# bcgsc/NanoSim

Measured on AMD Instinct MI355X. Metric: simulated reads/sec (genome mode, mean 8 kb), higher is better.
Workload: dtype u8

## Files before the change

nanosim_amd/csrc/nanosim_amd.hip:

```cpp
#include <hip/hip_runtime.h>
#include <hipcub/hipcub.hpp>
#include <stdio.h>
#include <stdlib.h>
#include <string.h>
#include <algorithm>
#include <chrono>
#include <atomic>
#include <condition_variable>
#include <functional>
#include <mutex>
#include <thread>
#include <type_traits>
#include <string>
#include <vector>

#include "ns_device.h"
#include "ns_materialise.h"
#include "ns_chain.h"
#include "ns_hp.h"
#include "ns_ir.h"
#include "ns_io.h"
#include "ns_pack.h"
#include "ns_cs_hist.h"
#include "ns_qual_hist.h"
// ... 201 lines not shown
        for (j = 0; j < NS_KDE_RETRY; ++j) {
            u32x4 w = ns_draw(key, ST_RATIO, 0, a, j, 0);
            double x = kde_sample(A.m.kde[NS_KDE_RATIO], w);
            if (0 <= x && x <= 1) { ratio = x; break; }
        }
        if (j == NS_KDE_RETRY) ratio = 0.5;
    }
    u32x4 ws = ns_draw(key, ST_STRAND, 0, a, 0, 0);
    ns_read rd;
    rd.rec_off = 0; rd.piece_off = piece_off; rd.n_pieces = (uint16_t)n_pieces;
    rd.reversed = (u32_to_p(ws.x) > A.m.strandness_rate) ? 1 : 0;
    if (meta_al) rd.reversed = (uint8_t)A.m_reversed;
    rd.flags = ok ? 1 : 3;
    rd.head = 0; rd.tail = 0;
    if (remainder != 0) {
        rd.head = (uint32_t)(int64_t)rint((double)remainder * ratio);
        rd.tail = (uint32_t)remainder - rd.head;
    }
    rd.seq_len = 0; rd.attempts = a;
    A.reads[r] = rd;
    cap = (cap + 3ull) & ~3ull;
    if (A.attempt > 0 && !meta_al && !trx_tab) A.l_cap[tid] = cap;
    if (A.attempt == 0 || meta_al || trx_tab) {
        A.ev_cap[r] = cap;
        if (n_pieces > 1u) A.sort_key[r] = 0x80000000u | ord_coarse(work) << 5 | ord_coarse(work0);
        else A.sort_key[r] = work > 0x7fffffffull ? 0x7fffffffu : (uint32_t)work;
        A.sort_idx[r] = (uint32_t)r;
    }
}

__device__ __forceinline__ unsigned long long wave_sum(unsigned long long v) {
    for (int off = 32; off > 0; off >>= 1) v += __shfl_xor(v, off);
    return v;
}

#ifndef NS_UCOOP_ITER
#define NS_UCOOP_ITER 3
#endif
#ifndef NS_UCOOP_MINW
#define NS_UCOOP_MINW 4
#endif
#ifndef NS_CHAIN_BLOCK
#define NS_CHAIN_BLOCK 256
#endif
#ifndef NS_CHAIN_BLOCK_BIG
#define NS_CHAIN_BLOCK_BIG 512
#endif
#define NS_PIECE_SLOTS 6u
#ifndef NS_CHAIN_MINW
#define NS_CHAIN_MINW 5
#endif
#ifdef NS_CHAIN_CLOCK
__device__ unsigned long long g_chain_clock[16];
#endif
template <bool LDS_TABLES, bool COOP, bool PIECES = false>
__global__ void __launch_bounds__(COOP ? 64 : NS_CHAIN_BLOCK_BIG, COOP ? (LDS_TABLES ? NS_UCOOP_MINW : 4) : NS_CHAIN_MINW) k_chain(GenArgs A) {
    extern __shared__ uint64_t lds_tbl[];
    CoopLds *coop = nullptr;
    if constexpr (COOP && !LDS_TABLES) { __shared__ CoopLds coop_lds; coop = &coop_lds; }
    Tabs T;
    if (LDS_TABLES) {
        const uint32_t nw = COOP ? A.m.ct.n_words_mix : A.m.ct.n_words_lds;
        for (uint32_t i = threadIdx.x; i < nw; i += blockDim.x) lds_tbl[i] = A.m.chain_blob[i];
        __syncthreads();
        T.w = lds_tbl;
    } else T.w = A.m.chain_blob;
    Tabs TM = T;
    if constexpr (COOP && !LDS_TABLES) {
        if (A.coop_mix) {
            for (uint32_t i = threadIdx.x; i < A.m.ct.n_words_mix; i += blockDim.x) lds_tbl[i] = A.m.chain_blob[i];
            __syncthreads();
            TM.w = lds_tbl;
        }
    }
    const ChainTab &ct = A.m.ct;
    const uint32_t lane = threadIdx.x & 63u;
    const uint64_t tid = COOP ? (uint64_t)blockIdx.x : (uint64_t)blockIdx.x * blockDim.x + threadIdx.x;
    const bool lead = COOP ? lane == 0 : true;
    const ns_params &prm = A.prm;
    if (!COOP && A.prio_thr) {
        uint32_t w = 0;
        if (tid < A.list_n) {
            const uint32_t k = A.sort_key[A.list[tid + (tid >= A.hole_at ? A.hole_len : 0u)]];
            w = (k >> 31) ? ord_coarse_floor((k >> 5) & 31u) : k;
        }
        for (int off = 32; off > 0; off >>= 1) w = max(w, (uint32_t)__shfl_xor((int)w, off));
        w = (uint32_t)__builtin_amdgcn_readfirstlane((int)w);
        if (w >= A.prio_thr[1]) __builtin_amdgcn_s_setprio(3);
        else if (w >= A.prio_thr[2]) __builtin_amdgcn_s_setprio(2);
        else if (w >= A.prio_thr[3]) __builtin_amdgcn_s_setprio(1);
    }
    else if (COOP || (PIECES && A.piece_mode == 1u) || blockIdx.x < (gridDim.x >> 6)) __builtin_amdgcn_s_setprio(3);
    else if (blockIdx.x < (gridDim.x >> 4)) __builtin_amdgcn_s_setprio(2);
    else if (blockIdx.x < (gridDim.x >> 2)) __builtin_amdgcn_s_setprio(1);
#ifdef NS_CHAIN_CLOCK
    const unsigned long long clk0 = wall_clock64(); uint32_t clk_multi = 0; unsigned long long clk_al = 0, clk_gap = 0, clk_pos = 0;
#endif
    unsigned long long st_over = 0, st_bases = 0, st_ref = 0, st_ev = 0;
    uint32_t st_max = 0;
    const bool piece_only = PIECES && !COOP && A.piece_mode == 1u;
    const uint32_t slot = piece_only ? (uint32_t)(tid / A.list_n) : 0u;
    const uint64_t li = piece_only ? tid % A.list_n : tid;
    if (piece_only ? slot < NS_PIECE_SLOTS : tid < A.list_n) {
        const uint64_t r = A.list ? A.list[li + (li >= A.hole_at ? A.hole_len : 0u)] : A.list_base + li;
        const int kind = (int)prm.kind;
        const bool trx_al = prm.trx && kind != NS_KIND_UNALIGNED;
        const bool meta_al = (A.meta && kind != NS_KIND_UNALIGNED) || trx_al;
        const ns_key key = make_key(A, trx_al ? trx_key_rel(A, r) : r);
        const uint32_t a = trx_al ? trx_attempt(A, r) : meta_al ? A.attempt : A.att_base[r] + A.attempt;
        ns_read rd = A.reads[r];
        const uint32_t n_pieces = rd.n_pieces;
#ifdef NS_CHAIN_CLOCK
        clk_multi = n_pieces > 1u;
#endif
        ns_piece *pc = A.pieces + rd.piece_off;
        uint32_t epoch = meta_al ? 0u : A.rstate[r] & 0xffffu, fails = meta_al ? 0u : A.rstate[r] >> 16;
        bool accepted = false, overflow = false;
        do {
            if (rd.flags & 2) { ++epoch; fails = 0; break; }
            const uint64_t ev_off = A.l_off ? A.l_base + A.l_off[tid] : A.ev_base + A.ev_off[r];
            const uint64_t ev_cap64 = A.l_off ? A.l_off[tid + 1] - A.l_off[tid] : A.ev_off[r + 1] - A.ev_off[r];
            const uint32_t ev_cap = ev_cap64 > 0xffffffffull ? 0xffffffffu : (uint32_t)ev_cap64;
            EvSink32 sink; sink.last_ins_len = 0; sink.overflow = false; sink.range = false; sink.stride = blockDim.x;
            int64_t total = (int64_t)rd.head + rd.tail;
            uint32_t evn = 0, evp = 0;
            const uint32_t trx_chrom = trx_al ? pc[0].pos : 0u;
            const uint32_t pi_lo = piece_only ? slot : 0u, pi_hi = (piece_only && slot + 1u < NS_PIECE_SLOTS) ? min(slot + 1u, n_pieces) : n_pieces;
            for (uint32_t pi = pi_lo; pi < pi_hi; ++pi) {
                ns_piece p = pc[pi];
                if (PIECES && !COOP && A.piece_mode == 2u) {
                    const uint32_t fl = (uint32_t)(p.ref_gpos >> 32);
                    if (fl & 1u) sink.range = true;
                    if (fl & 2u) sink.overflow = true;
                    p.ev_off = ev_off + p.ev_off;
                    pc[pi] = p;
                    evn += p.n_ev;
                    if (!p.kind) total += (int64_t)(int32_t)(uint32_t)p.ref_gpos;
                    continue;
                }
                if (piece_only) {
                    evp = (uint32_t)p.ev_off;
                    const uint32_t end = pi + 1u < n_pieces ? (uint32_t)pc[pi + 1u].ev_off : ev_cap;
                    sink.range = false; sink.overflow = false;
                    sink.ev = A.events + ev_off + evp; sink.cap = end > evp ? end - evp : 0u;
                }
                const int32_t m32 = (int32_t)p.ref_len;
                const uint32_t sid = p.kind ? NS_GAP_SEG + (pi >> 1) : (pi >> 1);
                if (!piece_only) { sink.ev = A.events + ev_off + evp; sink.cap = ev_cap > evp ? ev_cap - evp : 0; }
                sink.n = 0; sink.shift = 0;
// ... 116 lines not shown
            }
            if (!pos_ok || (!A.hp && !trx_al && (seq_len < prm.min_len || seq_len > prm.max_len))) { ++epoch; fails = 0; break; }
            rd.flags = 0; rd.seq_len = (uint32_t)seq_len; rd.attempts = a;
            uint32_t nl = 0; bool first = true;
            for (uint32_t pi = 0; pi < n_pieces; ++pi) {
                ns_piece p = pc[pi];
                if (p.kind && kind == NS_KIND_ALIGNED) {
                    if (A.meta) nl += 5 + dec_digits(p.out_len);
                    continue;
                }
                if (!first) nl += 2;
                first = false;
                nl += (A.ref.name_off[p.chrom + 1] - A.ref.name_off[p.chrom] - 1) + 1 + dec_digits(p.pos) + dec_digits(p.ref_len);
            }
            nl += (kind == NS_KIND_UNALIGNED ? 11u : 9u) + (meta_al ? 0u : dec_digits(A.name_first + r)) + ir_name;
            if (kind == NS_KIND_ALIGNED && n_pieces > 1) nl += 9;
            nl += 2  + 1 + dec_digits(rd.head) + 1 + 1 + dec_digits(rd.tail + polya);
            uint64_t err_len = 0;
            if (prm.emit_errlog && !A.errlen_later) {
                for (uint32_t pi = 0; pi < n_pieces; ++pi) {
                    ns_piece p = pc[pi];
                    if (p.kind) continue;
                    const ns_event *ev = A.events + p.ev_off;
                    for (uint32_t j = 0; j < p.n_ev; ++j) {
                        ns_event e = ev[j];
                        err_len += nl + dec_digits(e.pos) + dec_digits(ns_ev_len(e.info)) + 2u * ns_ev_len(e.info) + 9u;
                    }
                }
            }
            if (lead) {
                A.name_len[r] = (uint16_t)nl;
                A.rec_len[r] = prm.emit_records ? (uint64_t)nl + 2 + (uint64_t)seq_len + 1 + (prm.fastq ? (uint64_t)seq_len + 3 : 0) : 0;
                A.err_len[r] = err_len;
                if (A.polya) A.polya[r] = (uint16_t)polya;
                if (A.ir_need) A.ir_need[r] = spliced ? ir_slot_bytes(pc[0].ref_len) : 0;
                if (meta_al) { A.accept[r] = 1ull | (uint64_t)n_pieces << 32; A.sort_key[r] = evn; }
                st_bases = A.hp ? 0ull : (unsigned long long)seq_len; st_ref = ref_bases; st_ev = evn; st_max = (uint32_t)seq_len;
                if (trx_al) st_bases = st_ref = st_ev = 0;
            }
            accepted = true;
        } while (false);
        if (lead && !piece_only) {
            if (overflow) st_over += 1;
            A.reads[r] = rd;
            if (meta_al) {  }
            else if (accepted) A.att_base[r] = a;
            if (!meta_al && !accepted && !overflow) {
                A.rstate[r] = (epoch & 0xffffu) | fails << 16;
                A.next_list[atomicAdd(A.next_n, 1u)] = (uint32_t)r;
            }
        }
    }
#ifdef NS_CHAIN_CLOCK
    if (!COOP && A.attempt == 0) {
        const unsigned long long dt = wall_clock64() - clk0;
        const bool any_multi = __ballot(clk_multi != 0) != 0;
        if ((threadIdx.x & 63) == 0) { unsigned long long *C = g_chain_clock + (any_multi ? 4 : 0); atomicMax(&C[0], dt); atomicAdd(&C[1], dt); atomicAdd(&C[2], 1ull);
                                       atomicMax(&C[3], (unsigned long long)blockIdx.x << 32 | dt);
                                       if (any_multi) { atomicAdd(&g_chain_clock[8], clk_al); atomicAdd(&g_chain_clock[9], clk_gap); atomicAdd(&g_chain_clock[10], clk_pos ? wall_clock64() - clk_pos : 0ull); } }
    }
#endif
    st_over = wave_sum(st_over); st_bases = wave_sum(st_bases); st_ref = wave_sum(st_ref); st_ev = wave_sum(st_ev);
    if (A.prm.kind == NS_KIND_UNALIGNED) for (int off = 32; off > 0; off >>= 1) st_max = max(st_max, (uint32_t)__shfl_xor((int)st_max, off));
    if ((threadIdx.x & 63) == 0) {
        unsigned long long *S = ns_stats_way(A.stats, blockIdx.x & (NS_STATS_WAYS - 1u));
        if (st_over) atomicAdd(&S[NS_STAT_OVER], st_over);
        if (st_bases) atomicAdd(&S[NS_STAT_BASES], st_bases);
        if (st_ref) atomicAdd(&S[NS_STAT_REF_BASES], st_ref);
        if (st_ev) atomicAdd(&S[NS_STAT_EVENTS], st_ev);
        if (A.prm.kind == NS_KIND_UNALIGNED && st_max) atomicMax(&S[NS_STAT_MAX_READ], (unsigned long long)st_max);
    }
}

__global__ void __launch_bounds__(64) k_stats_fold(unsigned long long *stats, uint32_t *zero_me) {
    if (threadIdx.x == 0 && zero_me) *zero_me = 0;
    unsigned long long *S = ns_stats_way(stats, threadIdx.x);
    constexpr int MAX = NS_STAT_MAX_READ;
    unsigned long long v[MAX + 1];
    #pragma unroll
    for (int k = 0; k <= MAX; ++k) { v[k] = S[k]; S[k] = 0; }
    #pragma unroll
    for (int k = 0; k < MAX; ++k) v[k] = wave_sum(v[k]);
    for (int off = 32; off > 0; off >>= 1) { const unsigned long long o = __shfl_xor(v[MAX], off); v[MAX] = o > v[MAX] ? o : v[MAX]; }
    if (threadIdx.x == 0) {
        #pragma unroll
        for (int k = 0; k < MAX; ++k) if (v[k]) atomicAdd(&stats[k], v[k]);
        if (v[MAX]) atomicMax(&stats[MAX], v[MAX]);
    }
}

#define NS_ORD_BINS 2048u
__device__ __forceinline__ uint32_t ord_bin(uint32_t key31) {
    if (key31 >> 31) return 1023u - (key31 & 1023u);
    const uint32_t key = key31;
    uint32_t v = key;
    if (key >= 32u) { const uint32_t e = 31u - (uint32_t)__clz((int)key); v = (e - 4u) * 32u + ((key >> (e - 5u)) & 31u); }
    return 1024u + 1023u - v;
}
__global__ void __launch_bounds__(1024) k_order_hist(const uint32_t *__restrict__ keys, uint32_t n, uint32_t *__restrict__ hist) {
    __shared__ uint32_t h[NS_ORD_BINS];
    h[threadIdx.x] = 0; h[threadIdx.x + 1024u] = 0;
    __syncthreads();
    for (uint32_t i = blockIdx.x * 1024u + threadIdx.x; i < n; i += gridDim.x * 1024u) atomicAdd(&h[ord_bin(keys[i])], 1u);
    __syncthreads();
    if (h[threadIdx.x]) atomicAdd(&hist[threadIdx.x], h[threadIdx.x]);
    if (h[threadIdx.x + 1024u]) atomicAdd(&hist[threadIdx.x + 1024u], h[threadIdx.x + 1024u]);
// ... 2649 lines not shown
                    n_coop = (cur_n - std::min(cur_n, n_multi)) >> kn.coop_shift;
                const uint32_t coop_at = (a == 0 && prm->kind == NS_KIND_ALIGNED) ? std::min(cur_n, n_multi) : 0u;
                uint32_t m_coop = 0;
                if (coop_at && n_coop) {
                    const bool piece_threads = lds && !kn.no_piece_threads;
                    const uint32_t sh = piece_threads ? (kn.coop_shift > 1u ? kn.coop_shift - 1u : 0u) : (kn.coop_shift > 5u ? kn.coop_shift - 5u : 0u);
                    m_coop = std::min(coop_at, std::max(coop_at >> sh, 64u));
                }
                if (n_coop) {
                    GenArgs B = A; B.list_n = n_coop + m_coop; B.list = cur + (m_coop ? 0u : coop_at);
                    if (m_coop) { B.hole_at = m_coop; B.hole_len = coop_at - m_coop; }
                    B.coop_k1 = kn.ucoop_k1 ? 1u : 0u;
                    if ((rc = launch_chain_coop(ctx, B, st))) return rc;
                    if (coop_at) { A.list = cur + m_coop; A.hole_at = coop_at - m_coop; A.hole_len = n_coop; } else A.list = cur + n_coop;
                    A.list_n = cur_n - n_coop - m_coop;
                }
                uint32_t n_pt = 0;
                if (a == 0 && lds && n_coop && coop_at > m_coop && !kn.no_piece_threads) {
                    if (!ctx->stream3) {
                        HIPCHK(hipStreamCreateWithFlags(&ctx->stream3, hipStreamNonBlocking));
                        HIPCHK(hipEventCreateWithFlags(&ctx->ev_join3, hipEventDisableTiming));
                    }
                    n_pt = coop_at - m_coop;
                    const uint32_t cb = ctx->chain_block;
                    GenArgs P = A; P.list = cur + m_coop; P.list_n = n_pt; P.hole_at = 0; P.hole_len = 0; P.prio_thr = nullptr;
                    const size_t lds_p = ctx->lds_bytes + (P.ev_stage ? cb * 32u : 0u);
                    HIPCHK(hipStreamWaitEvent(ctx->stream3, ctx->ev_fork, 0));
                    P.piece_mode = 1;
                    k_chain<true, false, true><<<dim3((unsigned)(((uint64_t)n_pt * NS_PIECE_SLOTS + cb - 1) / cb)), dim3(cb), lds_p, ctx->stream3>>>(P);
                    P.piece_mode = 2;
                    k_chain<true, false, true><<<dim3((n_pt + cb - 1) / cb), dim3(cb), lds_p, ctx->stream3>>>(P);
                    HIPCHK(hipGetLastError());
                    HIPCHK(hipEventRecord(ctx->ev_join3, ctx->stream3));
                    A.list = cur + coop_at + n_coop; A.hole_at = 0; A.hole_len = 0; A.list_n = cur_n - coop_at - n_coop;
                }
                if (a == 0 && n_multi && !n_pt && prm->kind == NS_KIND_ALIGNED) A.prio_thr = ctx->ord_bins.view<const uint32_t>() + 2 * NS_ORD_BINS;
                if ((rc = launch_chain(ctx, A, st))) return rc;
                if (n_coop) HIPCHK(hipStreamWaitEvent(st, ctx->ev_join, 0));
                if (n_pt) HIPCHK(hipStreamWaitEvent(st, ctx->ev_join3, 0));
                HIPCHK(hipEventRecord(ctx->evt[EV_CHAIN_END], st));
                if (ctx->gate_signal) ctx->gate_signal->store(1, std::memory_order_release);
                if ((rc = end_pass(ctx, A, retry, stats, ms_chain, info, overflow))) return rc;
                if (overflow) break;
                cur_n = (uint32_t)(stats[NS_STAT_NEXT_N] & 0xffffffffull);
                if (!cur_n) { pl.tot_cap = used; break; }
                if (a + 1 >= NS_MAX_ATTEMPT) return attempt_limit(ctx);
                cur = nxt; nxt = cur == list_b ? list_c : list_b;
            }
            info->ms_kernel[NS_K_EVENTS] = ms_chain;
#ifdef NS_CHAIN_CLOCK
            if (prm->kind == NS_KIND_ALIGNED) { unsigned long long c[16], z[16] = {0}; HIPCHK(hipMemcpyFromSymbol(c, HIP_SYMBOL(g_chain_clock), sizeof c)); HIPCHK(hipMemcpyToSymbol(HIP_SYMBOL(g_chain_clock), z, sizeof z));
              fprintf(stderr, "chain clock: lane 0 of the multi waves: aligned pieces %.3f ms, gaps %.3f ms, behind the lists %.3f ms (means) | ", c[6] ? c[8] * 1e-5 / c[6] : 0.0, c[6] ? c[9] * 1e-5 / c[6] : 0.0, c[6] ? c[10] * 1e-5 / c[6] : 0.0);
              fprintf(stderr, "chain clock: single waves %llu max %.3f ms mean %.3f ms (the group's last block: %llu) | multi waves %llu max %.3f ms mean %.3f ms (the group's last block: %llu) | ms_chain %.3f\n",
                  c[2], c[0] * 1e-5, c[2] ? c[1] * 1e-5 / c[2] : 0.0, c[3] >> 32, c[6], c[4] * 1e-5, c[6] ? c[5] * 1e-5 / c[6] : 0.0, c[7] >> 32, ms_chain); }
#endif
            if (!overflow) break;
        }
        if (A.ir_need && (rc = ir_splice(ctx, A, n))) return rc;
        if (!A.hp) break;
        if ((rc = hp_stage1(ctx, prm, A, n, pl.tot_pieces, stats, &pl.ms_hp))) return rc;
        if (!stats[NS_STAT_HP_FAILED]) break;
        if (hp_round >= (int)NS_MAX_ATTEMPT) return fail(ctx, NS_EINVAL, "reads keep failing the final length check in -k mode");
        A.keep_state = 1;
    }
    return NS_OK;
}

static int check_params(ns_ctx *ctx, const ns_params *prm) {
    if (!ctx->has_model || !ctx->has_ref) return fail(ctx, NS_ESTATE, "ns_generate before ns_load_model/ns_set_reference");
    if (prm->kind > NS_KIND_PERFECT) return fail(ctx, NS_EINVAL, "bad kind");
    if (prm->emit_records > NS_EMIT_SIZES) return fail(ctx, NS_EINVAL, "bad emit_records");
    if (prm->kind != NS_KIND_PERFECT && !(ctx->m.flags & NS_MODEL_HAS_ERRORS)) return fail(ctx, NS_EINVAL, "model has no error tables");
    if (prm->kind == NS_KIND_UNALIGNED && !prm->use_lognormal && !(ctx->m.flags & NS_MODEL_HAS_UNALIGNED))
        return fail(ctx, NS_EINVAL, "model has no unaligned-length KDE");
    if (prm->fastq && !(ctx->m.flags & NS_MODEL_HAS_QUALS)) return fail(ctx, NS_EINVAL, "model has no quality tables");
    if (prm->chimeric && !(ctx->m.flags & NS_MODEL_HAS_CHIMERIC)) return fail(ctx, NS_EINVAL, "model has no chimeric tables");
    if (prm->kmer_bias && prm->kind == NS_KIND_ALIGNED && !(ctx->m.flags & NS_MODEL_HAS_HP))
        return fail(ctx, NS_EINVAL, "-k needs the homopolymer model (-hp)");
    const bool meta_al = prm->meta && prm->kind != NS_KIND_UNALIGNED;
    if (prm->meta) {
        if (!ctx->nspecies) return fail(ctx, NS_ESTATE, "metagenome batch before ns_set_species");
        if (prm->kind == NS_KIND_PERFECT && prm->chimeric) return fail(ctx, NS_EINVAL, "perfect reads cannot be chimeric");
        if (meta_al && !ctx->has_abun) return fail(ctx, NS_ESTATE, "metagenome batch before ns_set_abundance");
        if (meta_al && prm->chimeric && !ctx->has_inflated) return fail(ctx, NS_EINVAL, "chimeric metagenome batch needs abun_inflated");
    }
    if (prm->trx) {
        if (!ctx->has_trx) return fail(ctx, NS_ESTATE, "transcriptome batch before ns_set_transcriptome");
        if (prm->meta || prm->chimeric || prm->use_lognormal) return fail(ctx, NS_EINVAL, "transcriptome batches are neither metagenome nor chimeric nor log-normal");
        if (prm->kind != NS_KIND_UNALIGNED && !(ctx->m.flags & NS_MODEL_HAS_KDE2D)) return fail(ctx, NS_EINVAL, "model has no 2-D KDE (_aligned_region_2d)");
    }
    if (prm->model_ir) {
        if (!prm->trx) return fail(ctx, NS_EINVAL, "model_ir is a transcriptome option");
        if (!ctx->has_ir) return fail(ctx, NS_ESTATE, "model_ir batch before ns_set_intron_retention");
    }
    if (prm->n_reads > 0x7ffffff0ull) return fail(ctx, NS_EINVAL, "batch too large (split into several calls)");
    if (prm->first_read + prm->n_reads >= (1ull << 40)) return fail(ctx, NS_EINVAL, "read index exceeds 2^40");
    return NS_OK;
}

static int batch_args(ns_ctx *ctx, const ns_params *prm, size_t n, GenArgs &A) {
    int rc;
    if ((rc = ensure_all(ctx, {{ctx->n_pieces, n + 1}, {ctx->piece_off, n + 1}, {ctx->ev_cap, n + 1}, {ctx->ev_off, n + 1},
                               {ctx->l_cap, n + 1}, {ctx->l_off, n + 1}, {ctx->rec_len, n + 1}, {ctx->rec_off, n + 1},
                               {ctx->err_len, n + 1}, {ctx->err_off, n + 1}, {ctx->name_len, n + 1}, {ctx->reads, n},
                               {ctx->stats, NS_STATS_BYTES}, {ctx->sort_key, n + 1}, {ctx->sort_idx, n + 1}, {ctx->sort_key_out, n + 1},
                               {ctx->order, n + 1}, {ctx->list_b, (n + 1) * 4}, {ctx->list_c, (n + 1) * 4}, {ctx->rstate, n + 1},
                               {ctx->att_base, n + 1}, {ctx->scr_len, n + 1}, {ctx->scr_off, n + 1}})))
// ... 514 lines not shown
```

nanosim_amd/csrc/ns_chain.h:

```cpp
#pragma once
#include "ns_device.h"

struct Tabs {
    const uint64_t *w;
    NS_DEV const double *d(uint32_t off) const { return reinterpret_cast<const double *>(w + off); }
    NS_DEV const uint64_t *q(uint32_t off) const { return w + off; }
    NS_DEV const uint16_t *h(uint32_t off) const { return reinterpret_cast<const uint16_t *>(w + off); }
    NS_DEV const uint32_t *u(uint32_t off) const { return reinterpret_cast<const uint32_t *>(w + off); }
    NS_DEV const int32_t *i(uint32_t off) const { return reinterpret_cast<const int32_t *>(w + off); }
};

template <class V>
NS_DEV int32_t ecdf_lookup_g(const double *__restrict__ hi, const V *__restrict__ vhi, uint32_t n,
                                                 double vlo0, const uint16_t *__restrict__ guide, uint32_t u) {
    double p = u32_to_p(u);
    uint32_t s = guide[guide_cell(u)];
    if (s < n) {
        const double h0 = hi[s], h1 = hi[min(s + 1, n - 1)];
        if (p > h0) {
            ++s;
            if (s < n && p > h1) { ++s; while (s < n && p > hi[s]) ++s; }
        }
    }
    if (s >= n) { s = n - 1; p = hi[s]; }
// ... 490 lines not shown
                        if (st - 1 > Lk) { ty[k][2] = NS_MIS; ln[k][2] = st - 1 - Lk; ne = 3; }
                    }
                } else {
                    if (!Lk) { ty[k][0] = NS_DEL; ln[k][0] = st; ne = 1; }
                    else {
                        ty[k][0] = NS_DEL; ln[k][0] = st > Lk ? st - Lk : 1u; ne = 1;
                        if (Lk > st - 1) { ty[k][1] = NS_INS; ln[k][1] = Lk - (st - 1); ne = 2; }
                    }
                }
            }
            bad |= ln[k][0] > NS_EV_LEN_MAX || ln[k][1] > NS_EV_LEN_MAX || ln[k][2] > NS_EV_LEN_MAX;
            ln[k][0] = min(ln[k][0], NS_EV_LEN_MAX); ln[k][1] = min(ln[k][1], NS_EV_LEN_MAX); ln[k][2] = min(ln[k][2], NS_EV_LEN_MAX);
            n_ev[k] = ne; n_loc[k] = n_lane; n_lane += ne;
        }
        const uint32_t d_incl = wave_incl_scan(d_lane);
        const uint32_t ne_incl = wave_incl_scan(n_lane | n_exec_l << 16);
        const uint32_t d_front = d_incl - d_lane, n_front = (ne_incl & 0xffffu) - n_lane;
        auto dsh = [](uint32_t t, uint32_t l) { return t == NS_INS ? l : t == NS_DEL ? 0u - l : 0u; };
        #pragma unroll
        for (int k = 0; k < K; ++k) {
            if (!n_ev[k]) continue;
            const uint32_t sh = (uint32_t)s.shift + (pend0 + (i_incl - i_lane) + i_loc[k] - L[k]) - (d_front + d_loc[k]);
            const uint32_t d0 = dsh(ty[k][0], ln[k][0]), d1 = n_ev[k] > 1 ? dsh(ty[k][1], ln[k][1]) : 0u;
            if (!ev_shift_fits((int32_t)sh) || (n_ev[k] > 1 && !ev_shift_fits((int32_t)(sh + d0))) || (n_ev[k] > 2 && !ev_shift_fits((int32_t)(sh + d0 + d1)))) bad = true;
            const uint32_t slot = s.n + n_front + n_loc[k];
            if (slot < s.cap) { ns_event e; e.pos = ps[k][0]; e.info = ns_ev_pack(ln[k][0], ty[k][0], (int32_t)sh); s.ev[slot] = e; }
            if (n_ev[k] > 1 && slot + 1 < s.cap) { ns_event e; e.pos = ps[k][1]; e.info = ns_ev_pack(ln[k][1], ty[k][1], (int32_t)(sh + d0)); s.ev[slot + 1] = e; }
            if (n_ev[k] > 2 && slot + 2 < s.cap) { ns_event e; e.pos = ps[k][2]; e.info = ns_ev_pack(ln[k][2], ty[k][2], (int32_t)(sh + d0 + d1)); s.ev[slot + 2] = e; }
        }
        const uint32_t ne_tot = (uint32_t)__builtin_amdgcn_readlane((int)ne_incl, 63);
        const uint32_t n_blk = ne_tot & 0xffffu, n_ran = ne_tot >> 16;
        const uint32_t del_tot = (uint32_t)__builtin_amdgcn_readlane((int)d_incl, 63), ins_tot = (uint32_t)__builtin_amdgcn_readlane((int)i_incl, 63);
        uint32_t adv_tot = (uint32_t)__builtin_amdgcn_readlane((int)a_incl, 63);
        if (n_ran < 64u * K) adv_tot = (uint32_t)__builtin_amdgcn_readlane((int)wave_incl_scan(a_exec), 63);
        if (s.n + n_blk > s.cap) s.overflow = true;
        s.n += n_blk;
        l_new += (int32_t)ins_tot - (int32_t)del_tot;
        uint32_t pend1 = pend0 + ins_tot;
        if (HAS) {
            const int jl = 63 - __clzll((long long)HAS);
            pend1 = (uint32_t)__shfl((int)run, jl) + ins_tot - (uint32_t)__shfl((int)i_incl, jl);
        }
        s.shift = (int32_t)((uint32_t)s.shift + (pend0 + ins_tot - pend1) - del_tot);
        pend0 = pend1;
        pos0 += adv_tot;
        if (n_ran < 64u * K || pos0 >= (uint32_t)m_ref) break;
    }
    if (__ballot(bad)) s.range = true;
    if ((int32_t)pos0 > middle_ref) { l_new += (int32_t)pos0 - middle_ref; middle_ref = (int32_t)pos0; }
    return EList32{l_new, middle_ref};
}

#define COOP_MAX_BINS 16u
struct CoopLds {
    uint32_t err_tab[64];
    uint16_t step_tab[64][4];
    uint32_t match_tab[64][COOP_MAX_BINS];
    ns_event ev_buf[64];
};

__device__ inline EList32 coop_error_list(const Tabs &TM, const Tabs &T, const ChainTab &c, int32_t m_ref, const ns_key &key, uint32_t seg,
                                          uint32_t attempt, EvSink32 &s, CoopLds &S, uint32_t lane) {
    int32_t l_new = m_ref, pos = 0, middle_ref = m_ref;
    int state = NS_ST_START;
    u32x4 w = ns_draw(key, ST_EVENT, seg, attempt, 0, 0);
    int32_t prev_match = ecdf_lookup_g(T.d(c.fm_hi), T.d(c.fm_vhi), c.fm_n, c.fm_vlo0, T.h(c.fm_guide), w.x);
    if (prev_match < 2) prev_match = 2;
    pos += prev_match;
    uint32_t it0 = 1;
    int32_t last_ins_pos = -1;
    const uint64_t *trans = TM.q(c.trans);
    const int32_t *bins = T.i(c.mm_bin);
    const uint32_t *seg_off = T.u(c.mm_seg_off);
    const uint8_t *bin_lut = reinterpret_cast<const uint8_t *>(T.w + c.mm_bin_lut);
    auto bin_of = [&](int32_t v) -> uint32_t {
        if ((uint32_t)v < 256u) return bin_lut[v];
        uint32_t b = 0;
        for (; b < c.mm_nbins; ++b)
            if (bins[2 * b] <= v && v < bins[2 * b + 1]) break;
        return b >= c.mm_nbins ? c.mm_nbins - 1 : b;
    };
    uint32_t pbin = bin_of(prev_match);
    while (pos < middle_ref) {
        {
            const u32x4 wi = ns_draw(key, ST_EVENT, seg, attempt, it0 + lane, 0);
            uint32_t eb = 0;
#pragma unroll
            for (int st = 0; st < 7; ++st) eb |= (uint32_t)trans_pick_u(trans + 3 * st, wi.x) << (2 * st);
            S.err_tab[lane] = eb;
#pragma unroll
            for (int t = 0; t < 3; ++t) S.step_tab[lane][t] = (uint16_t)run_length_t(TM, c, t, wi.y, wi.z);
            if (c.int_image) {
                const uint16_t *g16 = T.h(c.mm_g16);
                const uint64_t *gvf = T.q(c.mm_gv_full);
                const uint32_t cell = wi.w >> 16, nb = c.mm_nbins;
                const uint64_t uu = wi.w;
                for (uint32_t b0 = 0; b0 < nb; b0 += 4) {
                    uint32_t o[4], nc[4], s0[4];
                    uint64_t ga[4], gb[4];
#pragma unroll
                    for (uint32_t k = 0; k < 4; ++k) {
                        const uint32_t b = min(b0 + k, nb - 1u);
                        o[k] = seg_off[b]; nc[k] = seg_off[b + 1] - o[k];
                        s0[k] = g16[(size_t)b * 65536u + cell];
                    }
#pragma unroll
                    for (uint32_t k = 0; k < 4; ++k) {
                        const uint32_t sc = min(s0[k], nc[k] ? nc[k] - 1u : 0u);
                        ga[k] = gvf[o[k] + sc]; gb[k] = gvf[o[k] + sc + 1u];
                    }
#pragma unroll
                    for (uint32_t k = 0; k < 4; ++k) {
                        const uint32_t b = min(b0 + k, nb - 1u);
                        const uint32_t k0 = (s0[k] < nc[k] ? 1u : 0u) & (uu >= NS_G_THR(ga[k]) ? 1u : 0u);
                        const uint32_t k1 = k0 & (s0[k] + 1u < nc[k] ? 1u : 0u) & (uu >= NS_G_THR(gb[k]) ? 1u : 0u);
                        const uint64_t g = k0 ? gb[k] : ga[k];
                        int32_t v = (int32_t)(uint32_t)(g >> 35) - 1;
                        if (!((s0[k] + k0 < nc[k]) && !k1 && (g & NS_GV_UNIT)))
                            v = ecdf_lookup_gv(gvf + o[k], nc[k], T.h(c.mm_guide) + NS_GUIDE_CELLS * b, wi.w, T.q(c.sub2_full), T.d(c.mm_hi) + o[k], T.d(c.mm_vhi) + o[k], T.d(c.mm_vlo0)[b]);
                        if (b0 + k < nb) S.match_tab[lane][b0 + k] = (uint32_t)(uint16_t)v | bin_of(v) << 16 | bin_of(v == 0 ? 1 : v) << 24;
                    }
                }
            } else
            for (uint32_t b = 0; b < c.mm_nbins; ++b) {
                const uint32_t o = seg_off[b];
                const int32_t v = ecdf_lookup_g(T.d(c.mm_hi) + o, T.d(c.mm_vhi) + o, seg_off[b + 1] - o, T.d(c.mm_vlo0)[b], T.h(c.mm_guide) + NS_GUIDE_CELLS * b, wi.w);
                S.match_tab[lane][b] = (uint32_t)(uint16_t)v | bin_of(v) << 16 | bin_of(v == 0 ? 1 : v) << 24;
            }
        }
        __builtin_amdgcn_fence(__ATOMIC_ACQ_REL, "wavefront");
        __builtin_amdgcn_wave_barrier();
        uint32_t nl = 0;
        uint32_t i = 0;
        for (; i < 64 && pos < middle_ref; ++i) {
            const int error = (int)((S.err_tab[i] >> (2 * state)) & 3u);
            int32_t step = S.step_tab[i][error];
            if (error == NS_INS) l_new += step; else if (error == NS_DEL) l_new -= step;
            int32_t epos = pos;
            if (error != NS_INS) {
                pos += step;
                if (pos >= middle_ref) { l_new += pos - middle_ref; middle_ref = pos; }
            } else {
                if (last_ins_pos == pos && (nl > 0 || s.n > 0)) {
                    if (nl > 0) --nl; else --s.n;
                    s.shift -= (int32_t)s.last_ins_len;
                }
                last_ins_pos = pos;
            }
            {
                const uint32_t l = step > (int32_t)NS_EV_LEN_MAX ? NS_EV_LEN_MAX : (uint32_t)step;
                if (step > (int32_t)NS_EV_LEN_MAX || !ev_shift_fits(s.shift)) s.range = true;
                ns_event e; e.pos = (uint32_t)epos; e.info = ns_ev_pack(l, (uint32_t)error, s.shift);
                if (lane == 0) S.ev_buf[nl] = e;
                ++nl;
                if (error == NS_INS) { s.shift += (int32_t)l; s.last_ins_len = l; } else if (error == NS_DEL) s.shift -= (int32_t)l;
            }
            state = NS_ST_MIS + error;
            const uint32_t me = S.match_tab[i][pbin];
            step = (int32_t)(me & 0xffffu);
            pbin = (me >> 16) & 0xffu;
            if (prev_match == 0 && step == 0) { step = 1; pbin = me >> 24; }
            prev_match = step;
            if (pos + prev_match > middle_ref) { l_new += pos + prev_match - middle_ref; middle_ref = pos + prev_match; }
            pos += prev_match;
            if (prev_match == 0) state += 3;
            else last_ins_pos = -1;
        }
        __builtin_amdgcn_fence(__ATOMIC_ACQ_REL, "wavefront");
        __builtin_amdgcn_wave_barrier();
        if (lane < nl) {
            if (s.n + lane < s.cap) s.ev[s.n + lane] = S.ev_buf[lane];
        }
        if (s.n + nl > s.cap) s.overflow = true;
        s.n += nl;
        it0 += i;
        __builtin_amdgcn_fence(__ATOMIC_ACQ_REL, "wavefront");
        __builtin_amdgcn_wave_barrier();
    }
    return EList32{l_new, middle_ref};
}
```

Before: 126.5 million.

## Walk cooperative error list from VGPR lanes via readlane instead of LDS

Restructures the wave-per-read error-list generation. Each lane still evaluates one speculative row into LDS, but the serial walk now reads rows through register readlane from a transposed per-lane copy, and buffers events in lane registers instead of an LDS event buffer. The step table is packed into two words per row. The aim is to cut LDS round-trips and barriers on the serial critical path, at the cost of more register pressure and a 16-way unrolled walk. Clock instrumentation for the cooperative path is also added behind a debug macro.

```diff
diff --git a/nanosim_amd/csrc/nanosim_amd.hip b/nanosim_amd/csrc/nanosim_amd.hip
--- a/nanosim_amd/csrc/nanosim_amd.hip
+++ b/nanosim_amd/csrc/nanosim_amd.hip
@@ -277,6 +277,8 @@
 #endif
 #ifdef NS_CHAIN_CLOCK
 __device__ unsigned long long g_chain_clock[16];
+#define NS_COOP_CLOCK_N 4096u
+__device__ unsigned long long g_coop_clock[NS_COOP_CLOCK_N][4];
 #endif
 template <bool LDS_TABLES, bool COOP, bool PIECES = false>
 __global__ void __launch_bounds__(COOP ? 64 : NS_CHAIN_BLOCK_BIG, COOP ? (LDS_TABLES ? NS_UCOOP_MINW : 4) : NS_CHAIN_MINW) k_chain(GenArgs A) {
@@ -320,6 +322,7 @@
     else if (blockIdx.x < (gridDim.x >> 2)) __builtin_amdgcn_s_setprio(1);
 #ifdef NS_CHAIN_CLOCK
     const unsigned long long clk0 = wall_clock64(); uint32_t clk_multi = 0; unsigned long long clk_al = 0, clk_gap = 0, clk_pos = 0;
+    if constexpr (COOP && !LDS_TABLES) { if (lane == 0) coop->clk[0] = coop->clk[1] = coop->clk[2] = coop->clk[3] = 0; }
 #endif
     unsigned long long st_over = 0, st_bases = 0, st_ref = 0, st_ev = 0;
     uint32_t st_max = 0;
@@ -542,6 +545,9 @@
         }
     }
 #ifdef NS_CHAIN_CLOCK
+    if constexpr (COOP && !LDS_TABLES) {
+        if (lane == 0 && A.attempt == 0 && blockIdx.x < NS_COOP_CLOCK_N) for (int k = 0; k < 4; ++k) g_coop_clock[blockIdx.x][k] = coop->clk[k];
+    }
     if (!COOP && A.attempt == 0) {
         const unsigned long long dt = wall_clock64() - clk0;
         const bool any_multi = __ballot(clk_multi != 0) != 0;
@@ -3297,7 +3303,12 @@
             if (prm->kind == NS_KIND_ALIGNED) { unsigned long long c[16], z[16] = {0}; HIPCHK(hipMemcpyFromSymbol(c, HIP_SYMBOL(g_chain_clock), sizeof c)); HIPCHK(hipMemcpyToSymbol(HIP_SYMBOL(g_chain_clock), z, sizeof z));
               fprintf(stderr, "chain clock: lane 0 of the multi waves: aligned pieces %.3f ms, gaps %.3f ms, behind the lists %.3f ms (means) | ", c[6] ? c[8] * 1e-5 / c[6] : 0.0, c[6] ? c[9] * 1e-5 / c[6] : 0.0, c[6] ? c[10] * 1e-5 / c[6] : 0.0);
               fprintf(stderr, "chain clock: single waves %llu max %.3f ms mean %.3f ms (the group's last block: %llu) | multi waves %llu max %.3f ms mean %.3f ms (the group's last block: %llu) | ms_chain %.3f\n",
-                  c[2], c[0] * 1e-5, c[2] ? c[1] * 1e-5 / c[2] : 0.0, c[3] >> 32, c[6], c[4] * 1e-5, c[6] ? c[5] * 1e-5 / c[6] : 0.0, c[7] >> 32, ms_chain); }
+                  c[2], c[0] * 1e-5, c[2] ? c[1] * 1e-5 / c[2] : 0.0, c[3] >> 32, c[6], c[4] * 1e-5, c[6] ? c[5] * 1e-5 / c[6] : 0.0, c[7] >> 32, ms_chain);
+              static unsigned long long cc[NS_COOP_CLOCK_N][4]; HIPCHK(hipMemcpyFromSymbol(cc, HIP_SYMBOL(g_coop_clock), sizeof cc));
+              uint32_t w = 0; for (uint32_t k = 1; k < NS_COOP_CLOCK_N; ++k) if (cc[k][3] > cc[w][3]) w = k;
+              fprintf(stderr, "coop clock: wave-per-read wavefront %u with the most iterations (%llu): speculative %.3f ms, walk %.3f ms, flush %.3f ms\n",
+                  w, cc[w][3], cc[w][0] * 1e-5, cc[w][1] * 1e-5, cc[w][2] * 1e-5);
+              static const unsigned long long zz[NS_COOP_CLOCK_N][4] = {}; HIPCHK(hipMemcpyToSymbol(HIP_SYMBOL(g_coop_clock), zz, sizeof zz)); }
 #endif
             if (!overflow) break;
         }
diff --git a/nanosim_amd/csrc/ns_chain.h b/nanosim_amd/csrc/ns_chain.h
--- a/nanosim_amd/csrc/ns_chain.h
+++ b/nanosim_amd/csrc/ns_chain.h
@@ -566,97 +566,121 @@
 }
 
 #define COOP_MAX_BINS 16u
+#define COOP_ROW_RA 16u
+#define COOP_ROW_RB 17u
+#define COOP_ROW_WORDS 19u
 struct CoopLds {
-    uint32_t err_tab[64];
-    uint16_t step_tab[64][4];
-    uint32_t match_tab[64][COOP_MAX_BINS];
-    ns_event ev_buf[64];
+    uint32_t match_tab[64][COOP_ROW_WORDS];
+#ifdef NS_CHAIN_CLOCK
+    unsigned long long clk[4], clk_t;
+#endif
 };
-
-__device__ inline EList32 coop_error_list(const Tabs &TM, const Tabs &T, const ChainTab &c, int32_t m_ref, const ns_key &key, uint32_t seg,
-                                          uint32_t attempt, EvSink32 &s, CoopLds &S, uint32_t lane) {
-    int32_t l_new = m_ref, pos = 0, middle_ref = m_ref;
-    int state = NS_ST_START;
-    u32x4 w = ns_draw(key, ST_EVENT, seg, attempt, 0, 0);
-    int32_t prev_match = ecdf_lookup_g(T.d(c.fm_hi), T.d(c.fm_vhi), c.fm_n, c.fm_vlo0, T.h(c.fm_guide), w.x);
-    if (prev_match < 2) prev_match = 2;
-    pos += prev_match;
-    uint32_t it0 = 1;
-    int32_t last_ins_pos = -1;
+#ifdef NS_CHAIN_CLOCK
+#define NS_COOP_CLK(S, lane, k) do { if ((lane) == 0) { const unsigned long long t_ = wall_clock64(); (S).clk[k] += t_ - (S).clk_t; (S).clk_t = t_; } } while (0)
+#else
+#define NS_COOP_CLK(S, lane, k) do { } while (0)
+#endif
+
+NS_DEV uint32_t coop_bin_of(const Tabs &T, const ChainTab &c, int32_t v) {
+    if ((uint32_t)v < 256u) return reinterpret_cast<const uint8_t *>(T.w + c.mm_bin_lut)[v];
+    const int32_t *bins = T.i(c.mm_bin);
+    uint32_t b = 0;
+    for (; b < c.mm_nbins; ++b)
+        if (bins[2 * b] <= v && v < bins[2 * b + 1]) break;
+    return b >= c.mm_nbins ? c.mm_nbins - 1 : b;
+}
+NS_DEV uint32_t coop_match_word(const Tabs &T, const ChainTab &c, int32_t v) {
+    return (uint32_t)(uint16_t)v | coop_bin_of(T, c, v) << 16 | coop_bin_of(T, c, v == 0 ? 1 : v) << 24;
+}
+
+NS_DEV void coop_eval_row(const Tabs &TM, const Tabs &T, const ChainTab &c, const ns_key &key, uint32_t seg, uint32_t attempt, uint32_t it,
+                          uint32_t *row) {
     const uint64_t *trans = TM.q(c.trans);
-    const int32_t *bins = T.i(c.mm_bin);
     const uint32_t *seg_off = T.u(c.mm_seg_off);
-    const uint8_t *bin_lut = reinterpret_cast<const uint8_t *>(T.w + c.mm_bin_lut);
-    auto bin_of = [&](int32_t v) -> uint32_t {
-        if ((uint32_t)v < 256u) return bin_lut[v];
-        uint32_t b = 0;
-        for (; b < c.mm_nbins; ++b)
-            if (bins[2 * b] <= v && v < bins[2 * b + 1]) break;
-        return b >= c.mm_nbins ? c.mm_nbins - 1 : b;
-    };
-    uint32_t pbin = bin_of(prev_match);
-    while (pos < middle_ref) {
-        {
-            const u32x4 wi = ns_draw(key, ST_EVENT, seg, attempt, it0 + lane, 0);
-            uint32_t eb = 0;
+    const u32x4 wi = ns_draw(key, ST_EVENT, seg, attempt, it, 0);
+    uint32_t eb = 0;
 #pragma unroll
-            for (int st = 0; st < 7; ++st) eb |= (uint32_t)trans_pick_u(trans + 3 * st, wi.x) << (2 * st);
-            S.err_tab[lane] = eb;
+    for (int st = 0; st < 7; ++st) eb |= (uint32_t)trans_pick_u(trans + 3 * st, wi.x) << (2 * st);
+    row[COOP_ROW_RA] = eb | (uint32_t)(uint16_t)run_length_t(TM, c, NS_MIS, wi.y, wi.z) << 16;
+    row[COOP_ROW_RB] = (uint32_t)(uint16_t)run_length_t(TM, c, NS_INS, wi.y, wi.z) | (uint32_t)(uint16_t)run_length_t(TM, c, NS_DEL, wi.y, wi.z) << 16;
+    if (c.int_image) {
+        const uint16_t *g16 = T.h(c.mm_g16);
+        const uint64_t *gvf = T.q(c.mm_gv_full);
+        const uint32_t cell = wi.w >> 16, nb = c.mm_nbins;
+        const uint64_t uu = wi.w;
+        for (uint32_t b0 = 0; b0 < nb; b0 += 4) {
+            uint32_t o[4], nc[4], s0[4];
+            uint64_t ga[4], gb[4];
 #pragma unroll
-            for (int t = 0; t < 3; ++t) S.step_tab[lane][t] = (uint16_t)run_length_t(TM, c, t, wi.y, wi.z);
-            if (c.int_image) {
-                const uint16_t *g16 = T.h(c.mm_g16);
-                const uint64_t *gvf = T.q(c.mm_gv_full);
-                const uint32_t cell = wi.w >> 16, nb = c.mm_nbins;
-                const uint64_t uu = wi.w;
-                for (uint32_t b0 = 0; b0 < nb; b0 += 4) {
-                    uint32_t o[4], nc[4], s0[4];
-                    uint64_t ga[4], gb[4];
+            for (uint32_t k = 0; k < 4; ++k) {
+                const uint32_t b = min(b0 + k, nb - 1u);
+                o[k] = seg_off[b]; nc[k] = seg_off[b + 1] - o[k];
+                s0[k] = g16[(size_t)b * 65536u + cell];
+            }
 #pragma unroll
-                    for (uint32_t k = 0; k < 4; ++k) {
-                        const uint32_t b = min(b0 + k, nb - 1u);
-                        o[k] = seg_off[b]; nc[k] = seg_off[b + 1] - o[k];
-                        s0[k] = g16[(size_t)b * 65536u + cell];
-                    }
+            for (uint32_t k = 0; k < 4; ++k) {
+                const uint32_t sc = min(s0[k], nc[k] ? nc[k] - 1u : 0u);
+                ga[k] = gvf[o[k] + sc]; gb[k] = gvf[o[k] + sc + 1u];
+            }
 #pragma unroll
-                    for (uint32_t k = 0; k < 4; ++k) {
-                        const uint32_t sc = min(s0[k], nc[k] ? nc[k] - 1u : 0u);
-                        ga[k] = gvf[o[k] + sc]; gb[k] = gvf[o[k] + sc + 1u];
-                    }
-#pragma unroll
-                    for (uint32_t k = 0; k < 4; ++k) {
-                        const uint32_t b = min(b0 + k, nb - 1u);
-                        const uint32_t k0 = (s0[k] < nc[k] ? 1u : 0u) & (uu >= NS_G_THR(ga[k]) ? 1u : 0u);
-                        const uint32_t k1 = k0 & (s0[k] + 1u < nc[k] ? 1u : 0u) & (uu >= NS_G_THR(gb[k]) ? 1u : 0u);
-                        const uint64_t g = k0 ? gb[k] : ga[k];
-                        int32_t v = (int32_t)(uint32_t)(g >> 35) - 1;
-                        if (!((s0[k] + k0 < nc[k]) && !k1 && (g & NS_GV_UNIT)))
-                            v = ecdf_lookup_gv(gvf + o[k], nc[k], T.h(c.mm_guide) + NS_GUIDE_CELLS * b, wi.w, T.q(c.sub2_full), T.d(c.mm_hi) + o[k], T.d(c.mm_vhi) + o[k], T.d(c.mm_vlo0)[b]);
-                        if (b0 + k < nb) S.match_tab[lane][b0 + k] = (uint32_t)(uint16_t)v | bin_of(v) << 16 | bin_of(v == 0 ? 1 : v) << 24;
-                    }
-                }
-            } else
-            for (uint32_t b = 0; b < c.mm_nbins; ++b) {
-                const uint32_t o = seg_off[b];
-                const int32_t v = ecdf_lookup_g(T.d(c.mm_hi) + o, T.d(c.mm_vhi) + o, seg_off[b + 1] - o, T.d(c.mm_vlo0)[b], T.h(c.mm_guide) + NS_GUIDE_CELLS * b, wi.w);
-                S.match_tab[lane][b] = (uint32_t)(uint16_t)v | bin_of(v) << 16 | bin_of(v == 0 ? 1 : v) << 24;
+            for (uint32_t k = 0; k < 4; ++k) {
+                const uint32_t b = min(b0 + k, nb - 1u);
+                const uint32_t k0 = (s0[k] < nc[k] ? 1u : 0u) & (uu >= NS_G_THR(ga[k]) ? 1u : 0u);
+                const uint32_t k1 = k0 & (s0[k] + 1u < nc[k] ? 1u : 0u) & (uu >= NS_G_THR(gb[k]) ? 1u : 0u);
+                const uint64_t g = k0 ? gb[k] : ga[k];
+                int32_t v = (int32_t)(uint32_t)(g >> 35) - 1;
+                if (!((s0[k] + k0 < nc[k]) && !k1 && (g & NS_GV_UNIT)))
+                    v = ecdf_lookup_gv(gvf + o[k], nc[k], T.h(c.mm_guide) + NS_GUIDE_CELLS * b, wi.w, T.q(c.sub2_full), T.d(c.mm_hi) + o[k], T.d(c.mm_vhi) + o[k], T.d(c.mm_vlo0)[b]);
+                if (b0 + k < nb) row[b0 + k] = coop_match_word(T, c, v);
             }
         }
-        __builtin_amdgcn_fence(__ATOMIC_ACQ_REL, "wavefront");
-        __builtin_amdgcn_wave_barrier();
-        uint32_t nl = 0;
-        uint32_t i = 0;
-        for (; i < 64 && pos < middle_ref; ++i) {
-            const int error = (int)((S.err_tab[i] >> (2 * state)) & 3u);
-            int32_t step = S.step_tab[i][error];
+    } else
+    for (uint32_t b = 0; b < c.mm_nbins; ++b) {
+        const uint32_t o = seg_off[b];
+        const int32_t v = ecdf_lookup_g(T.d(c.mm_hi) + o, T.d(c.mm_vhi) + o, seg_off[b + 1] - o, T.d(c.mm_vlo0)[b], T.h(c.mm_guide) + NS_GUIDE_CELLS * b, wi.w);
+        row[b] = coop_match_word(T, c, v);
+    }
+}
+
+NS_DEV uint32_t coop_tr_row(uint32_t lane, uint32_t r) { return 16u * (lane >> 4) + r; }
+NS_DEV uint32_t coop_tr_col(uint32_t lane) { return lane & 15u; }
+
+#ifndef NS_COOP_COUNT
+#define NS_COOP_COUNT(what)
+#endif
+enum { NS_CCNT_POP_EARLIER, NS_CCNT_ZERO_RULE };
+struct CoopChain {
+    int32_t l_new, pos, middle_ref, prev_match, last_ins_pos;
+    uint32_t state, pbin;
+};
+template <uint32_t N> struct CoopIdx { static constexpr uint32_t value = N; };
+template <class W>
+struct CoopRows {
+    typename W::Reg ra, rb;
+    typename W::Reg col[COOP_MAX_BINS];
+};
+template <class W>
+NS_DEV uint32_t coop_walk_block(const CoopRows<W> &R, CoopChain &k, EvSink32 &s, typename W::Reg &ev_pos, typename W::Reg &ev_info, uint32_t &nl_out) {
+    int32_t l_new = k.l_new, pos = k.pos, middle_ref = k.middle_ref, prev_match = k.prev_match, last_ins_pos = k.last_ins_pos;
+    uint32_t state = k.state, pbin = k.pbin;
+    uint32_t nl = 0;
+    uint32_t n_it = 0;
+    auto one = [&](uint32_t g, auto rc) __attribute__((always_inline)) -> bool {
+            constexpr uint32_t r = decltype(rc)::value;
+            if (pos >= middle_ref) return false;
+            const uint32_t i = g + r;
+            const uint32_t wa = W::rd(R.ra, i), wb = W::rd(R.rb, i);
+            const uint32_t me = W::rd(R.col[r], g + pbin);
+            const int error = (int)((wa >> (2u * state)) & 3u);
+            int32_t step = (int32_t)(error == NS_MIS ? wa >> 16 : error == NS_INS ? wb & 0xffffu : wb >> 16);
             if (error == NS_INS) l_new += step; else if (error == NS_DEL) l_new -= step;
-            int32_t epos = pos;
+            const int32_t epos = pos;
             if (error != NS_INS) {
                 pos += step;
                 if (pos >= middle_ref) { l_new += pos - middle_ref; middle_ref = pos; }
             } else {
                 if (last_ins_pos == pos && (nl > 0 || s.n > 0)) {
-                    if (nl > 0) --nl; else --s.n;
+                    if (nl > 0) --nl; else { --s.n; NS_COOP_COUNT(NS_CCNT_POP_EARLIER); }
                     s.shift -= (int32_t)s.last_ins_len;
                 }
                 last_ins_pos = pos;
@@ -664,32 +688,92 @@
             {
                 const uint32_t l = step > (int32_t)NS_EV_LEN_MAX ? NS_EV_LEN_MAX : (uint32_t)step;
                 if (step > (int32_t)NS_EV_LEN_MAX || !ev_shift_fits(s.shift)) s.range = true;
-                ns_event e; e.pos = (uint32_t)epos; e.info = ns_ev_pack(l, (uint32_t)error, s.shift);
-                if (lane == 0) S.ev_buf[nl] = e;
+                W::wr(ev_pos, nl, (uint32_t)epos);
+                W::wr(ev_info, nl, ns_ev_pack(l, (uint32_t)error, s.shift));
                 ++nl;
                 if (error == NS_INS) { s.shift += (int32_t)l; s.last_ins_len = l; } else if (error == NS_DEL) s.shift -= (int32_t)l;
             }
-            state = NS_ST_MIS + error;
-            const uint32_t me = S.match_tab[i][pbin];
+            state = NS_ST_MIS + (uint32_t)error;
             step = (int32_t)(me & 0xffffu);
             pbin = (me >> 16) & 0xffu;
-            if (prev_match == 0 && step == 0) { step = 1; pbin = me >> 24; }
+            if (prev_match == 0 && step == 0) { step = 1; pbin = me >> 24; NS_COOP_COUNT(NS_CCNT_ZERO_RULE); }
             prev_match = step;
             if (pos + prev_match > middle_ref) { l_new += pos + prev_match - middle_ref; middle_ref = pos + prev_match; }
             pos += prev_match;
             if (prev_match == 0) state += 3;
             else last_ins_pos = -1;
-        }
+            ++n_it;
+            return true;
+    };
+    for (uint32_t g = 0; g < 64u; g += 16u)
+        if (!(one(g, CoopIdx<0>{}) && one(g, CoopIdx<1>{}) && one(g, CoopIdx<2>{}) && one(g, CoopIdx<3>{}) && one(g, CoopIdx<4>{}) && one(g, CoopIdx<5>{}) &&
+              one(g, CoopIdx<6>{}) && one(g, CoopIdx<7>{}) && one(g, CoopIdx<8>{}) && one(g, CoopIdx<9>{}) && one(g, CoopIdx<10>{}) && one(g, CoopIdx<11>{}) &&
+              one(g, CoopIdx<12>{}) && one(g, CoopIdx<13>{}) && one(g, CoopIdx<14>{}) && one(g, CoopIdx<15>{}))) break;
+    k.l_new = l_new; k.pos = pos; k.middle_ref = middle_ref; k.prev_match = prev_match; k.last_ins_pos = last_ins_pos;
+    k.state = state; k.pbin = pbin;
+    nl_out = nl;
+    return n_it;
+}
+NS_DEV void coop_flush_lane(const EvSink32 &s, uint32_t nl, uint32_t lane, uint32_t pos, uint32_t info) {
+    if (lane < nl && s.n + lane < s.cap) { ns_event e; e.pos = pos; e.info = info; s.ev[s.n + lane] = e; }
+}
+NS_DEV void coop_flush_close(EvSink32 &s, uint32_t nl) {
+    if (s.n + nl > s.cap) s.overflow = true;
+    s.n += nl;
+}
+NS_DEV CoopChain coop_chain_open(const Tabs &T, const ChainTab &c, int32_t m_ref, const ns_key &key, uint32_t seg, uint32_t attempt) {
+    CoopChain k;
+    k.l_new = m_ref; k.pos = 0; k.middle_ref = m_ref; k.state = NS_ST_START; k.last_ins_pos = -1;
+    const u32x4 w = ns_draw(key, ST_EVENT, seg, attempt, 0, 0);
+    k.prev_match = ecdf_lookup_g(T.d(c.fm_hi), T.d(c.fm_vhi), c.fm_n, c.fm_vlo0, T.h(c.fm_guide), w.x);
+    if (k.prev_match < 2) k.prev_match = 2;
+    k.pos += k.prev_match;
+    k.pbin = coop_bin_of(T, c, k.prev_match);
+    return k;
+}
+
+#ifndef NS_HOST_TEST
+struct CoopWave {
+    typedef uint32_t Reg;
+    static __device__ __forceinline__ uint32_t rd(Reg v, uint32_t lane) { return (uint32_t)__builtin_amdgcn_readlane((int)v, (int)lane); }
+    static __device__ __forceinline__ void wr(Reg &v, uint32_t lane, uint32_t x) {
+        v = __builtin_amdgcn_mbcnt_hi(~0u, __builtin_amdgcn_mbcnt_lo(~0u, 0u)) == lane ? x : v;
+    }
+};
+__device__ __forceinline__ int32_t coop_uni(int32_t v) { return __builtin_amdgcn_readfirstlane(v); }
+
+__device__ inline EList32 coop_error_list(const Tabs &TM, const Tabs &T, const ChainTab &c, int32_t m_ref, const ns_key &key, uint32_t seg,
+                                          uint32_t attempt, EvSink32 &s, CoopLds &S, uint32_t lane) {
+    CoopChain k = coop_chain_open(T, c, m_ref, key, seg, attempt);
+    k.l_new = coop_uni(k.l_new); k.pos = coop_uni(k.pos); k.middle_ref = coop_uni(k.middle_ref); k.prev_match = coop_uni(k.prev_match);
+    k.pbin = (uint32_t)coop_uni((int32_t)k.pbin);
+    s.n = (uint32_t)coop_uni((int32_t)s.n); s.shift = coop_uni(s.shift); s.last_ins_len = (uint32_t)coop_uni((int32_t)s.last_ins_len);
+    uint32_t it0 = 1;
+#ifdef NS_CHAIN_CLOCK
+    if (lane == 0) S.clk_t = wall_clock64();
+#endif
+    while (k.pos < k.middle_ref) {
+        CoopRows<CoopWave> R;
+        coop_eval_row(TM, T, c, key, seg, attempt, it0 + lane, S.match_tab[lane]);
         __builtin_amdgcn_fence(__ATOMIC_ACQ_REL, "wavefront");
         __builtin_amdgcn_wave_barrier();
-        if (lane < nl) {
-            if (s.n + lane < s.cap) s.ev[s.n + lane] = S.ev_buf[lane];
-        }
-        if (s.n + nl > s.cap) s.overflow = true;
-        s.n += nl;
-        it0 += i;
+        R.ra = S.match_tab[lane][COOP_ROW_RA]; R.rb = S.match_tab[lane][COOP_ROW_RB];
+#pragma unroll
+        for (uint32_t r = 0; r < COOP_MAX_BINS; ++r) R.col[r] = S.match_tab[coop_tr_row(lane, r)][coop_tr_col(lane)];
         __builtin_amdgcn_fence(__ATOMIC_ACQ_REL, "wavefront");
         __builtin_amdgcn_wave_barrier();
-    }
-    return EList32{l_new, middle_ref};
-}
+        NS_COOP_CLK(S, lane, 0);
+        uint32_t ev_pos = 0, ev_info = 0, nl;
+        const uint32_t n_it = coop_walk_block<CoopWave>(R, k, s, ev_pos, ev_info, nl);
+        NS_COOP_CLK(S, lane, 1);
+        coop_flush_lane(s, nl, lane, ev_pos, ev_info);
+        coop_flush_close(s, nl);
+        it0 += n_it;
+        NS_COOP_CLK(S, lane, 2);
+#ifdef NS_CHAIN_CLOCK
+        if (lane == 0) S.clk[3] += n_it;
+#endif
+    }
+    return EList32{k.l_new, k.middle_ref};
+}
+#endif
```

Result: no change. 126.8 million, median of 3 (+0.2%).
